# 2646207530/hamer-yolo

Measured on AMD Instinct MI355X. Metric: hands/sec (HaMeR ViT-H/16 + decoder + MANO forward; detector bypassed), higher is better.
Workload: dtype fp16; 1 GPU; BASELINE configs[1]: batch=64 synthetic 256x256 crops per GPU, HaMeR ViT-H/16 + 6-layer decoder + MANO, 16-bit MFMA (fp16 operands), crops resident in HBM; batch_per_gpu=64, global_batch=64, batches_in_flight=2, weights=seeded random-init fp32 master weights, rounded to the operand type at load, parallelism=crop-shard x1

## Files before the change

hamer_yolo_amd/csrc/decoder.hip:

```cpp
#include "common.h"
#include "hamer_hip_internal.h"

namespace {

__global__ __launch_bounds__(256) void linear_f32_kernel(const float* __restrict__ x, int ldx,
                                                         const float* __restrict__ W, int ldw,
                                                         const float* __restrict__ bias, const float* resid, int ldr,
                                                         float* out, int ldo, int M, int N, int K, int act) {
  __shared__ f32x4_t part[4][64];
  const int lane = threadIdx.x & 63, wave = threadIdx.x >> 6;
  const int n0 = blockIdx.x * 16, m0 = blockIdx.y * 16;
  const int g = lane >> 4, li = lane & 15;
  int mr = m0 + li; mr = mr < M ? mr : M - 1;
  int nr = n0 + li; nr = nr < N ? nr : N - 1;
  const float* xp = x + (size_t)mr * ldx + 4 * g;
  const float* wp = W + (size_t)nr * ldw + 4 * g;
  f32x4_t acc = f32x4_t{0.f, 0.f, 0.f, 0.f};
  constexpr int PF = 4;
  int kb = wave * 16;
  for (; kb + 64 * (PF - 1) < K; kb += 64 * PF) {
    f32x4_t xv[PF], wv[PF];
#pragma unroll
    for (int p = 0; p < PF; ++p) { xv[p] = *(const f32x4_t*)(xp + kb + 64 * p); wv[p] = *(const f32x4_t*)(wp + kb + 64 * p); }
#pragma unroll
    for (int p = 0; p < PF; ++p)
#pragma unroll
      for (int i = 0; i < 4; ++i) acc = __builtin_amdgcn_mfma_f32_16x16x4f32(wv[p][i], xv[p][i], acc, 0, 0, 0);
  }
  for (; kb < K; kb += 64) {
    const f32x4_t xv = *(const f32x4_t*)(xp + kb);
    const f32x4_t wv = *(const f32x4_t*)(wp + kb);
#pragma unroll
    for (int i = 0; i < 4; ++i) acc = __builtin_amdgcn_mfma_f32_16x16x4f32(wv[i], xv[i], acc, 0, 0, 0);
  }
  part[wave][lane] = acc;
  __syncthreads();
  if (wave != 0) return;
  f32x4_t v = (part[0][lane] + part[1][lane]) + (part[2][lane] + part[3][lane]);
  const int m = m0 + li, n = n0 + 4 * g;
  if (m >= M || n >= N) return;
  if (bias) v += *(const f32x4_t*)(bias + n);
  if (act == 1) {
#pragma unroll
    for (int r = 0; r < 4; ++r) v[r] = gelu_erf(v[r]);
  }
  if (resid) v += *(const f32x4_t*)(resid + (size_t)m * ldr + n);
  *(f32x4_t*)(out + (size_t)m * ldo + n) = v;
}

constexpr int CA_MAXT = 256;

template <class E>
__global__ __launch_bounds__(64) void cross_attention_kernel(const float* __restrict__ q, const E* __restrict__ kv,
                                                             int ldkv, int k_off, int v_off, float* __restrict__ out,
                                                             int B, int tokens, int heads, float scale) {
  __shared__ float ps[CA_MAXT];
  __shared__ float qs[64];
  typedef __attribute__((ext_vector_type(8))) E vec8;
  const int lane = threadIdx.x;
  const int b = blockIdx.x / heads, h = blockIdx.x % heads;
  const int inner = heads * 64;
  qs[lane] = q[(size_t)b * inner + h * 64 + lane];
  __syncthreads();
  const E* kbase = kv + (size_t)b * tokens * ldkv + k_off + h * 64;
// ... 19 lines not shown
        }
      sc[i] = (d0 + d1) * scale;
      mx = fmaxf(mx, sc[i]);
    }
  }
  mx = wave_max(mx);
  float sum = 0.f;
#pragma unroll
  for (int i = 0; i < CA_MAXT / 64; ++i) {
    const int t = lane + 64 * i;
    if (t < tokens) {
      float p;
      if constexpr (sizeof(E) == 4) p = expf(sc[i] - mx);
      else p = __expf(sc[i] - mx);
      ps[t] = p;
      sum += p;
    }
  }
  sum = wave_sum(sum);
  __syncthreads();
  float o[4] = {0.f, 0.f, 0.f, 0.f};
  int t = 0;
  for (; t + 8 <= tokens; t += 8) {
    float v[8];
#pragma unroll
    for (int j = 0; j < 8; ++j) v[j] = (float)vbase[(size_t)(t + j) * ldkv + lane];
#pragma unroll
    for (int j = 0; j < 8; ++j) o[j & 3] = fmaf(ps[t + j], v[j], o[j & 3]);
  }
  for (; t < tokens; ++t) o[0] = fmaf(ps[t], (float)vbase[(size_t)t * ldkv + lane], o[0]);
  out[(size_t)b * inner + h * 64 + lane] = ((o[0] + o[1]) + (o[2] + o[3])) / sum;
}

__global__ void split_head_kernel(const float* __restrict__ head, int ldh, float* __restrict__ pose6d,
                                  float* __restrict__ betas, float* __restrict__ cam, int B) {
  const int i = blockIdx.x * 256 + threadIdx.x;
  if (i >= B * 109) return;
  const int b = i / 109, c = i % 109;
  const float v = head[(size_t)b * ldh + c];
  if (c < 96) pose6d[b * 96 + c] = v;
  else if (c < 106) betas[b * 10 + (c - 96)] = v;
  else cam[b * 3 + (c - 106)] = v;
}

}

extern "C" int hm_linear_f32(const float* x, int ldx, const float* W, int ldw, const float* bias, const float* resid,
                             int ldr, float* out, int ldo, int M, int N, int K, int act, void* stream_) {
  if (!x || !W || !out || M <= 0 || N <= 0 || K <= 0) return hm_set_error(HM_ERR_ARG, "hm_linear_f32: bad arguments");
  if (K % 16 != 0 || N % 4 != 0 || ldx % 4 != 0 || ldw % 4 != 0 || ldo % 4 != 0 || (resid && ldr % 4 != 0))
    return hm_set_error(HM_ERR_ARG, "hm_linear_f32: K % 16, N % 4 and ld % 4 must be 0");
  if (ldx < K || ldw < K || ldo < N) return hm_set_error(HM_ERR_ARG, "hm_linear_f32: leading dimension too small");
  if (((uintptr_t)x | (uintptr_t)W | (uintptr_t)out | (uintptr_t)bias | (uintptr_t)resid) & 15)
    return hm_set_error(HM_ERR_ARG, "hm_linear_f32: pointers must be 16-byte aligned");
  dim3 grid((N + 15) / 16, (M + 15) / 16), block(256);
  HmProfScope prof(HM_K_LINEAR_F32, act, M, N, K, (hipStream_t)stream_);
  hipLaunchKernelGGL(linear_f32_kernel, grid, block, 0, (hipStream_t)stream_, x, ldx, W, ldw, bias, resid, ldr, out, ldo,
                     M, N, K, act);
  return hm_check_launch("hm_linear_f32");
}

extern "C" int hm_cross_attention(const float* q, const void* kv, int ldkv, int k_off, int v_off, float* out, int B,
                                  int tokens, int heads, int dim_head, float scale, int dtype, void* stream_) {
  if (!q || !kv || !out || B <= 0 || heads <= 0) return hm_set_error(HM_ERR_ARG, "hm_cross_attention: bad arguments");
  if (dim_head != 64 || tokens <= 0 || tokens > CA_MAXT)
    return hm_set_error(HM_ERR_ARG, "hm_cross_attention: dim_head must be 64 and tokens <= 256");
  if (ldkv % 8 != 0 || k_off % 8 != 0 || v_off % 8 != 0 || ((uintptr_t)kv & 15))
    return hm_set_error(HM_ERR_ARG, "hm_cross_attention: kv rows must be 16-byte aligned");
  if (dtype == HM_DTYPE_F32 && ((uintptr_t)kv & 31)) return hm_set_error(HM_ERR_ARG, "hm_cross_attention: fp32 kv rows must be 32-byte aligned");
  dim3 grid(B * heads), block(64);
  hipStream_t s = (hipStream_t)stream_;
  HmProfScope prof(HM_K_CROSS_ATTN, 0, B, tokens, heads, s);
  if (dtype == HM_DTYPE_BF16)
    hipLaunchKernelGGL(cross_attention_kernel<__bf16>, grid, block, 0, s, q, (const __bf16*)kv, ldkv, k_off, v_off, out, B, tokens, heads, scale);
  else if (dtype == HM_DTYPE_F16)
    hipLaunchKernelGGL(cross_attention_kernel<_Float16>, grid, block, 0, s, q, (const _Float16*)kv, ldkv, k_off, v_off, out, B, tokens, heads, scale);
  else if (dtype == HM_DTYPE_F32)
    hipLaunchKernelGGL(cross_attention_kernel<float>, grid, block, 0, s, q, (const float*)kv, ldkv, k_off, v_off, out, B, tokens, heads, scale);
  else
    return hm_set_error(HM_ERR_ARG, "hm_cross_attention: bad dtype");
  return hm_check_launch("hm_cross_attention");
}

int hm_split_head(const float* head, int ldh, float* pose6d, float* betas, float* cam, int B, hipStream_t s) {
  hipLaunchKernelGGL(split_head_kernel, dim3((B * 109 + 255) / 256), dim3(256), 0, s, head, ldh, pose6d, betas, cam, B);
  return hm_check_launch("hm_split_head");
}
```

hamer_yolo_amd/csrc/forward.hip:

```cpp
#include "common.h"
#include <stdlib.h>
#include "hamer_hip_internal.h"

int hm_split_head(const float* head, int ldh, float* pose6d, float* betas, float* cam, int B, hipStream_t s);

namespace {

inline size_t align256(size_t x) { return (x + 255) & ~(size_t)255; }

struct Layout {
  size_t patches, x, h, qkv, att, mlp, kv, xd, hd, t1, t2, head, stats, rowstats, hs, mlps, atts, partials, total;
  size_t x2, tsize, tmetric, tindex;
  int ksplit_proj, ksplit_fc2;
};

int pick_split_k(int M, int N, int K) {
  const int tiles = ((M + 127) / 128) * ((N + 127) / 128), nk = K / 64;
  if (M > 2048 || N < 512 || K % 64 != 0 || tiles * 2 > 256) return 1;
  int want = 256 / tiles;
  if (want > 8) want = 8;
  if (want > nk) want = nk;
  while (want > 1 && nk % want != 0) --want;
  return want;
}
// ... 253 lines not shown
      }
      HM_TRY(hm_layernorm_mx8(x, b.ln2_g, b.ln2_b, h, hs, M, D, w->vit_eps, stream));
      HM_TRY(gemm8(h, hs, D, b.fc1_w8, b.fc1_ws, w->mlp_dim, mlp, w->mlp_dim, b.fc1_b, HM_EPI_GELU_MX8, nullptr, mlps));
      HM_TRY(gemm8(mlp, mlps, w->mlp_dim, b.fc2_w8, b.fc2_ws, D, x, D, b.fc2_b, HM_EPI_RESID_F32, x, nullptr));
    } else if (fold) {
      HM_TRY(gemm(h, D, b.qkv_w, D, 3 * D, qkv, 3 * D, b.qkv_bias_ln, HM_EPI_LN_STORE, nullptr, 0, 0, b.qkv_colsum));
      HM_TRY(hm_vit_attention(qkv, att, B, tokens, w->heads, D / w->heads, scale, dt, stream));
      HM_TRY(gemm(att, D, b.proj_w, D, D, x, D, b.proj_b, HM_EPI_RESID_LN, x, D, 0, b.ln2_g));
      HM_TRY(gemm(h, D, b.fc1_w, D, w->mlp_dim, mlp, w->mlp_dim, b.fc1_bias_ln, HM_EPI_LN_GELU, nullptr, 0, 0, b.fc1_colsum));
      if (i + 1 < w->depth) HM_TRY(gemm(mlp, w->mlp_dim, b.fc2_w, w->mlp_dim, D, x, D, b.fc2_b, HM_EPI_RESID_LN, x, D, 0, w->blocks[i + 1].ln1_g));
      else HM_TRY(gemm(mlp, w->mlp_dim, b.fc2_w, w->mlp_dim, D, x, D, b.fc2_b, HM_EPI_RESID_F32, x, D, 0));
    } else {
      if (i == 0) {
        HM_TRY(hm_layernorm(x, b.ln1_g, b.ln1_b, h, dt, M, D, w->vit_eps, stream));
        HM_TRY(probe(h, D, M, 0, D, 0));
      }
      HM_TRY(gemm(h, D, b.qkv_w, D, 3 * D, qkv, 3 * D, b.qkv_b, HM_EPI_STORE, nullptr, 0, 0));
      for (int c = 0; c < 3; ++c) HM_TRY(probe(qkv, 3 * D, M, c * D, D, 6 * i + 1 + c));
      HM_TRY(hm_vit_attention(qkv, att, B, tokens, w->heads, D / w->heads, b.attn_scale_mul != 0.f ? scale * b.attn_scale_mul : scale, dt, stream));
      HM_TRY(resid_gemm_ln(att, D, b.proj_w, b.proj_b, L.ksplit_proj, b.ln2_g, b.ln2_b, h));
      HM_TRY(probe(h, D, M, 0, D, 6 * i + 4));
      HM_TRY(gemm(h, D, b.fc1_w, D, w->mlp_dim, mlp, w->mlp_dim, b.fc1_b, HM_EPI_GELU, nullptr, 0, 0, nullptr, b.gelu_out_scale));
      HM_TRY(probe(mlp, w->mlp_dim, M, 0, w->mlp_dim, 6 * i + 5));
      const bool last = i + 1 == w->depth;
      HM_TRY(resid_gemm_ln(mlp, w->mlp_dim, b.fc2_w, b.fc2_b, L.ksplit_fc2, last ? w->last_g : w->blocks[i + 1].ln1_g,
                           last ? w->last_b : w->blocks[i + 1].ln1_b, last ? tok : h));
      HM_TRY(probe(last ? tok : h, D, M, 0, D, 6 * (i + 1)));
    }
  }
  if (fold || fp8) HM_TRY(hm_layernorm(x, w->last_g, w->last_b, tok, dt, M, D, w->vit_eps, stream));
  }

  const int dim = w->dec_dim, inner = w->dec_heads * w->dec_dim_head, ldkv = w->dec_depth * 2 * inner;
  {
    hm_gemm_args g{};
    g.X = tok; g.W = w->kv_w; g.C = kv; g.M = B * ctx_tokens; g.N = ldkv; g.K = D; g.ldx = D; g.ldw = D; g.ldc = ldkv;
    g.epilogue = dt == HM_DTYPE_F32 ? HM_EPI_F32 : HM_EPI_STORE; g.dtype = dt;
    if (dt == HM_DTYPE_F32) HM_TRY(hm_gemm_f32(&g, stream));
    else HM_TRY(hm_gemm(&g, stream));
    for (int i = 0; i < w->dec_depth; ++i) {
      HM_TRY(probe(kv, ldkv, B * ctx_tokens, i * 2 * inner, inner, 6 * w->depth + 1 + 2 * i));
      HM_TRY(probe(kv, ldkv, B * ctx_tokens, i * 2 * inner + inner, inner, 6 * w->depth + 2 + 2 * i));
    }
  }
  float *xd = (float*)(ws + L.xd), *hd = (float*)(ws + L.hd), *t1 = (float*)(ws + L.t1), *t2 = (float*)(ws + L.t2);
  HM_TRY(hm_broadcast_rows(w->token0, xd, B, dim, stream));
  const float dscale = 1.0f / sqrtf((float)w->dec_dim_head);
  for (int i = 0; i < w->dec_depth; ++i) {
    const hm_dec_layer& l = w->layers[i];
    HM_TRY(hm_layernorm(xd, l.ln0_g, l.ln0_b, hd, HM_OUT_F32, B, dim, w->dec_eps, stream));
    if (l.sa_w) {
      HM_TRY(hm_linear_f32(hd, dim, l.sa_w, dim, l.sa_out_b, xd, dim, xd, dim, B, dim, dim, 0, stream));
    } else {
      HM_TRY(hm_linear_f32(hd, dim, l.sa_v_w, dim, nullptr, nullptr, 0, t1, inner, B, inner, dim, 0, stream));
      HM_TRY(hm_linear_f32(t1, inner, l.sa_out_w, inner, l.sa_out_b, xd, dim, xd, dim, B, dim, inner, 0, stream));
    }
    HM_TRY(hm_layernorm(xd, l.ln1_g, l.ln1_b, hd, HM_OUT_F32, B, dim, w->dec_eps, stream));
    HM_TRY(hm_linear_f32(hd, dim, l.ca_q_w, dim, nullptr, nullptr, 0, t1, inner, B, inner, dim, 0, stream));
    HM_TRY(hm_cross_attention(t1, kv, ldkv, i * 2 * inner, i * 2 * inner + inner, t2, B, ctx_tokens, w->dec_heads,
                              w->dec_dim_head, l.ca_scale_mul != 0.f ? dscale * l.ca_scale_mul : dscale, dt, stream));
    HM_TRY(hm_linear_f32(t2, inner, l.ca_out_w, inner, l.ca_out_b, xd, dim, xd, dim, B, dim, inner, 0, stream));
    HM_TRY(hm_layernorm(xd, l.ln2_g, l.ln2_b, hd, HM_OUT_F32, B, dim, w->dec_eps, stream));
    HM_TRY(hm_linear_f32(hd, dim, l.ff1_w, dim, l.ff1_b, nullptr, 0, t1, w->dec_mlp, B, w->dec_mlp, dim, 1, stream));
    HM_TRY(hm_linear_f32(t1, w->dec_mlp, l.ff2_w, w->dec_mlp, l.ff2_b, xd, dim, xd, dim, B, dim, w->dec_mlp, 0, stream));
  }
  float* head = (float*)(ws + L.head);
  HM_TRY(hm_linear_f32(xd, dim, w->head_w, dim, w->head_b, nullptr, 0, head, 112, B, 112, dim, 0, stream));
  HM_TRY(hm_split_head(head, 112, out->pose6d, out->betas, out->cam, B, (hipStream_t)stream));
  return hm_mano_forward(&w->mano, out->pose6d, out->betas, out->cam, out->rotmats, out->verts, out->joints, out->cam_t,
                         out->kp2d, B, w->focal_length, w->image_size, stream);
}
```

hamer_yolo_amd/csrc/status.hip:

```cpp
#include <stdio.h>
#include <string.h>
#include "common.h"
#include "hamer_hip_internal.h"

static thread_local char g_err[512] = "";

int hm_set_error(int code, const char* msg) {
  snprintf(g_err, sizeof(g_err), "%s", msg ? msg : "");
  return code;
}

int hm_check_launch(const char* what) {
  hipError_t e = hipGetLastError();
  if (e == hipSuccess) return HM_OK;
  snprintf(g_err, sizeof(g_err), "%s: %s", what, hipGetErrorString(e));
  return HM_ERR_HIP;
}

int hm_device_cu_count(void) {
  static std::mutex mu;
  static int cus[64] = {0};
  int dev = 0;
  if (hipGetDevice(&dev) != hipSuccess) return -1;
  std::lock_guard<std::mutex> lock(mu);
  if (dev < 64 && cus[dev] > 0) return cus[dev];
  int n = 0;
  if (hipDeviceGetAttribute(&n, hipDeviceAttributeMultiprocessorCount, dev) != hipSuccess) return -1;
  if (dev < 64) cus[dev] = n;
  return n;
}

#include <atomic>
static std::atomic<int> g_opts[HM_OPT_COUNT];
int hm_option(int key) {
  return (key >= 0 && key < HM_OPT_COUNT) ? g_opts[key].load(std::memory_order_relaxed) : 0;
}
extern "C" int hm_get_option(int key) { return hm_option(key); }
extern "C" int hm_option_count(void) { return HM_OPT_COUNT; }
extern "C" int hm_set_option(int key, int value) {
  if (key < 0 || key >= HM_OPT_COUNT) return hm_set_error(HM_ERR_ARG, "hm_set_option: unknown key");
  if (value < 0) return hm_set_error(HM_ERR_ARG, "hm_set_option: value must be >= 0");
  if ((key == HM_OPT_PX_GRID || key == HM_OPT_FP8P_GRID) && value != 0 && (value < 8 || value % 8 != 0))
    return hm_set_error(HM_ERR_ARG, "hm_set_option: a persistent grid is 0 (default) or a multiple of the 8 XCDs");
  if (key == HM_OPT_GEMM_STAGGER && value > 4)
    return hm_set_error(HM_ERR_ARG, "hm_set_option: HM_OPT_GEMM_STAGGER is 0 (default), 1 (lockstep), 2 (staggered), 3 or 4 (one kernel staggered)");
  g_opts[key].store(value, std::memory_order_relaxed);
  return HM_OK;
}

extern "C" int hm_version(void) { return HM_VERSION; }
extern "C" const char* hm_last_error_string(void) { return g_err; }
```

hamer_yolo_amd/lib.py:

```python
from __future__ import annotations

import ctypes as C
import os

HERE = os.path.dirname(os.path.abspath(__file__))
LIB_PATH = os.path.join(HERE, "libhamer_hip.so")

HM_DTYPE_BF16, HM_DTYPE_F16, HM_OUT_F32 = 0, 1, 2
HM_DTYPE_F32 = 2
HM_EPI_STORE, HM_EPI_GELU, HM_EPI_RESID_F32, HM_EPI_F32, HM_EPI_SILU = 0, 1, 2, 3, 4
HM_EPI_RESID_LN, HM_EPI_LN_STORE, HM_EPI_LN_GELU, HM_EPI_GELU_MX8 = 5, 6, 7, 8
HM_VERSION = 402
OPTION_NAMES = ("HM_OPT_PX_GRID", "HM_OPT_FP8P_GRID", "HM_OPT_FP8_ONE_TILE", "HM_OPT_FP8P_RESID", "HM_OPT_TOME_NO_SPLITK",
                "HM_OPT_TOME_SCALAR_ATTENTION", "HM_OPT_RESID_IN_EPILOGUE", "HM_OPT_CONV_TILE", "HM_OPT_CONV_SPLITK",
                "HM_OPT_PX_LDS_EPILOGUE", "HM_OPT_CONV_DIRECT", "HM_OPT_GEMM_TILE_RULE", "HM_OPT_CONV_KGROUPS",
                "HM_OPT_CONV_GENERAL_LOADER", "HM_OPT_CONV_STEM_PAIR", "HM_OPT_ATT_GRID", "HM_OPT_GEMM_STAGGER")
globals().update({_n: _i for _i, _n in enumerate(OPTION_NAMES)})

EXPORTS = [
    "hm_version", "hm_last_error_string", "hm_gemm", "hm_layernorm", "hm_vit_attention", "hm_patch_im2col",
    "hm_linear_f32", "hm_broadcast_rows", "hm_cross_attention", "hm_mano_forward", "hm_crop_box_from_bbox",
    "hm_crop_batch", "hm_hamer_workspace_bytes", "hm_hamer_forward", "hm_prof_begin", "hm_prof_collect", "hm_prof_end",
    "hm_conv2d_nhwc", "hm_conv2d_stem_pair", "hm_maxpool_nhwc", "hm_upsample2x_nhwc", "hm_letterbox_plan_make", "hm_letterbox_tables",
    "hm_letterbox", "hm_yolo_decode", "hm_nms_workspace_bytes", "hm_yolo_nms", "hm_yolo_run", "hm_gemm_set_variant", "hm_gemm_set_group_m", "hm_ln_finalize", "hm_layernorm_accum", "hm_gemm_fp8", "hm_layernorm_mx8", "hm_vit_attention_mx8", "hm_nchw3_to_nhwc8", "hm_gap_linear",
    "hm_tome_index_bytes", "hm_tome_attention", "hm_tome_merge", "hm_set_option", "hm_get_option", "hm_tome_merge_metric", "hm_conv_splitk_bytes", "hm_yolo_decode_batch", "hm_letterbox_batch",
    "hm_option_count", "hm_gemm_px_grid", "hm_absmax16", "hm_mesh_overlay_workspace_bytes", "hm_mesh_overlay",
    "hm_sar_saigb", "hm_sar_graph_mix", "hm_sar_linear", "hm_sar_softargmax", "hm_sar_postprocess",
    "hm_conv2d_f32_relu", "hm_nchw3_to_nhwc8_f32", "hm_gap_linear_f32", "hm_sar_saigb_f32", "hm_sar_graph_mix_f32", "hm_sar_linear_f32",
    "hm_gemm_f32", "hm_vit_attention_f32",
    "hm_dwconv7_ln", "hm_ln_patchify2", "hm_stem4_im2col", "hm_sar_saigb_ch",
    "hm_mesh_render_workspace_bytes", "hm_mesh_render",
    "hm_attention_grid",
    "hm_crop_aa_box_from_bbox", "hm_crop_batch_aa",
    "hm_pose_eval",
    "hm_skeleton_overlay_workspace_bytes", "hm_skeleton_overlay",
    "hm_det_match", "hm_det_ap_workspace_bytes", "hm_det_ap", "hm_det_ap_curve",
    "hm_nms_batch_workspace_bytes", "hm_yolo_nms_batch",
    "hm_tta_sizes", "hm_tta_tables", "hm_tta_scale", "hm_yolo_decode_batch_tta",
    "hm_mesh_score", "hm_pck_auc_workspace_bytes", "hm_pck_auc",
    "hm_mask_score_workspace_bytes", "hm_mask_score",
]
KIND_NAMES = ["gemm", "layernorm", "attention", "im2col", "linear_f32", "cross_attn", "mano", "crop", "conv", "other"]


class HipLibraryError(RuntimeError):
    pass


vp, fp = C.c_void_p, C.c_void_p


class GemmArgs(C.Structure):
    _fields_ = [("X", vp), ("W", vp), ("C", vp), ("bias", vp), ("resid", vp),
                ("M", C.c_int), ("N", C.c_int), ("K", C.c_int),
                ("ldx", C.c_int), ("ldw", C.c_int), ("ldc", C.c_int), ("ldr", C.c_int),
                ("resid_mod", C.c_int), ("epilogue", C.c_int), ("dtype", C.c_int),
                ("ln_gamma", vp), ("ln_xg", vp), ("ln_stats", vp), ("ln_colsum", vp), ("k_split", C.c_int), ("out_scale", C.c_float)]


class GemmFp8Args(C.Structure):
    _fields_ = [("X8", vp), ("x_scales", vp), ("W8", vp), ("w_scale", vp), ("C", vp), ("bias", vp), ("resid", vp),
                ("out_scales", vp), ("M", C.c_int), ("N", C.c_int), ("K", C.c_int), ("ldx", C.c_int), ("ldw", C.c_int),
                ("ldc", C.c_int), ("ldr", C.c_int), ("epilogue", C.c_int), ("out_dtype", C.c_int)]


class ManoModel(C.Structure):
    _fields_ = [("v_template", vp), ("shapedirs", vp), ("posedirs", vp), ("J_regressor", vp), ("lbs_weights", vp),
                ("n_verts", C.c_int)]


class CropBox(C.Structure):
    _fields_ = [("m0", C.c_double), ("m4", C.c_double), ("x0", C.c_int32), ("y0", C.c_int32),
                ("flip", C.c_int32), ("reserved", C.c_int32)]
# ... 97 lines not shown
class HamerOutputs(C.Structure):
    _fields_ = [(n, vp) for n in ("pose6d", "betas", "cam", "rotmats", "verts", "joints", "cam_t", "kp2d", "tokens")]


_lib = None


def load() -> C.CDLL:
    global _lib
    if _lib is not None:
        return _lib
    if not os.path.exists(LIB_PATH):
        raise HipLibraryError(
            f"{LIB_PATH} not found: build it with `python -m hamer_yolo_amd.build` (hipcc, gfx950). "
            "There is no CPU fallback for the hot path.")
    try:
        import torch
    except ImportError:
        pass
    try:
        lib = C.CDLL(LIB_PATH)
    except OSError as e:
        raise HipLibraryError(f"cannot load {LIB_PATH}: {e}") from e
    i, f, d = C.c_int, C.c_float, C.c_double
    lib.hm_version.restype = i
    lib.hm_last_error_string.restype = C.c_char_p
    lib.hm_gemm.argtypes = [C.POINTER(GemmArgs), vp]
    lib.hm_layernorm.argtypes = [vp, vp, vp, vp, i, i, i, f, vp]
    lib.hm_vit_attention.argtypes = [vp, vp, i, i, i, i, f, i, vp]
    lib.hm_patch_im2col.argtypes = [vp, vp, i, i, i, i, i, i, i, i, vp]
    lib.hm_linear_f32.argtypes = [vp, i, vp, i, vp, vp, i, vp, i, i, i, i, i, vp]
    lib.hm_broadcast_rows.argtypes = [vp, vp, i, i, vp]
    lib.hm_cross_attention.argtypes = [vp, vp, i, i, i, vp, i, i, i, i, f, i, vp]
    lib.hm_mano_forward.argtypes = [C.POINTER(ManoModel), vp, vp, vp, vp, vp, vp, vp, vp, i, f, f, vp]
    lib.hm_crop_box_from_bbox.argtypes = [d, d, d, i, i, C.POINTER(CropBox)]
    lib.hm_crop_batch.argtypes = [vp, i, i, vp, vp, i, i, C.POINTER(C.c_float), C.POINTER(C.c_float), vp]
    lib.hm_crop_aa_box_from_bbox.argtypes = [d, d, d, i, i, C.POINTER(CropAaBox), C.POINTER(C.c_float)]
    lib.hm_crop_batch_aa.argtypes = [vp, i, i, vp, vp, vp, i, i, C.POINTER(C.c_float), C.POINTER(C.c_float), vp]
    lib.hm_hamer_workspace_bytes.argtypes = [C.POINTER(HamerWeights), i]
    lib.hm_hamer_workspace_bytes.restype = C.c_size_t
    lib.hm_hamer_forward.argtypes = [C.POINTER(HamerWeights), vp, i, C.POINTER(HamerOutputs), vp, C.c_size_t, vp]
    lib.hm_ln_finalize.argtypes = [vp, vp, i, i, C.c_float, vp]
    lib.hm_gemm_fp8.argtypes = [C.POINTER(GemmFp8Args), vp]
    lib.hm_layernorm_mx8.argtypes = [vp, vp, vp, vp, vp, i, i, C.c_float, vp]
    lib.hm_vit_attention_mx8.argtypes = [vp, vp, vp, i, i, i, i, C.c_float, vp]
    lib.hm_nchw3_to_nhwc8.argtypes = [vp, vp, i, i, i, i, vp]
    lib.hm_gap_linear.argtypes = [vp, i, i, vp, C.c_float, vp, vp, i, i, vp]
    lib.hm_layernorm_accum.argtypes = [vp, vp, i, vp, vp, vp, vp, i, i, i, C.c_float, vp]
    lib.hm_absmax16.argtypes = [vp, i, i, i, i, i, vp, vp]
    lib.hm_conv2d_nhwc.argtypes = [C.POINTER(ConvArgs), vp]
    lib.hm_conv_splitk_bytes.argtypes = [C.POINTER(ConvArgs)]
    lib.hm_conv2d_stem_pair.argtypes = [C.POINTER(ConvArgs), C.POINTER(ConvArgs), vp]
    lib.hm_conv_splitk_bytes.restype = C.c_size_t
    lib.hm_maxpool_nhwc.argtypes = [vp, i, vp, i, i, i, i, i, i, i, i, i, vp]
    lib.hm_upsample2x_nhwc.argtypes = [vp, i, vp, i, i, i, i, i, i, vp]
    lib.hm_letterbox_plan_make.argtypes = [i, i, i, i, C.POINTER(LetterboxPlan)]
    lib.hm_letterbox_tables.argtypes = [C.POINTER(LetterboxPlan), C.POINTER(C.c_int32)]
    lib.hm_letterbox.argtypes = [vp, C.POINTER(LetterboxPlan), vp, vp, i, vp, vp]
    lib.hm_letterbox_batch.argtypes = [vp, C.c_size_t, i, C.POINTER(LetterboxPlan), vp, vp, i, vp]
    lib.hm_yolo_decode.argtypes = [vp, i, vp, i, i, i, i, f, C.POINTER(C.c_float), vp]
    lib.hm_yolo_decode_batch.argtypes = [vp, i, vp, i, i, i, i, f, C.POINTER(C.c_float), i, C.c_size_t, vp]
    lib.hm_tta_sizes.argtypes = [i, i, d, i, C.POINTER(C.c_int)]
    lib.hm_tta_tables.argtypes = [i, i, d, i, i, C.POINTER(C.c_int32)]
    lib.hm_tta_scale.argtypes = [vp, vp, vp, i, i, i, d, i, i, vp]
    lib.hm_yolo_decode_batch_tta.argtypes = [vp, i, vp, i, i, i, i, f, C.POINTER(C.c_float), i, C.c_size_t, f, i, f, vp]
    lib.hm_nms_workspace_bytes.argtypes = [i]
# ... 137 lines not shown
```

include/hamer_hip.h:

```cpp
#ifndef HAMER_HIP_H
#define HAMER_HIP_H
#include <stddef.h>
#include <stdint.h>

#ifdef __cplusplus
extern "C" {
#endif

#define HM_VERSION 402

enum { HM_DTYPE_BF16 = 0, HM_DTYPE_F16 = 1,
       HM_DTYPE_F32 = 2  };

enum {
  HM_EPI_STORE = 0,
  HM_EPI_GELU = 1,
  HM_EPI_RESID_F32 = 2,
  HM_EPI_F32 = 3,
  HM_EPI_SILU = 4,
  HM_EPI_RESID_LN = 5,
  HM_EPI_LN_STORE = 6,
  HM_EPI_LN_GELU = 7,
  HM_EPI_GELU_MX8 = 8,
  HM_EPI_RELU = 9,
// ... 11 lines not shown
  int resid_mod;
  int epilogue;
  int dtype;
  const float* ln_gamma;
  void* ln_xg;
  float* ln_stats;
  const float* ln_colsum;
  int k_split;
  float out_scale;
} hm_gemm_args;

int hm_gemm(const hm_gemm_args* args, void* stream);
int hm_ln_finalize(const float* partials, float* row_stats, int M, int D, float eps, void* stream);
int hm_gemm_set_variant(int variant);
int hm_gemm_set_group_m(int group_m);
enum {
  HM_OPT_PX_GRID = 0,
  HM_OPT_FP8P_GRID = 1,
  HM_OPT_FP8_ONE_TILE = 2,
  HM_OPT_FP8P_RESID = 3,
  HM_OPT_TOME_NO_SPLITK = 4,
  HM_OPT_TOME_SCALAR_ATTENTION = 5,
  HM_OPT_RESID_IN_EPILOGUE = 6,
  HM_OPT_CONV_TILE = 7,
  HM_OPT_CONV_SPLITK = 8,
  HM_OPT_PX_LDS_EPILOGUE = 9,
  HM_OPT_CONV_DIRECT = 10,
  HM_OPT_GEMM_TILE_RULE = 11,
  HM_OPT_CONV_KGROUPS = 12,
  HM_OPT_CONV_GENERAL_LOADER = 13,
  HM_OPT_CONV_STEM_PAIR = 14,
  HM_OPT_ATT_GRID = 15,
  HM_OPT_GEMM_STAGGER = 16,
  HM_OPT_COUNT = 17
};
int hm_set_option(int key, int value);
int hm_get_option(int key);
int hm_option_count(void);
int hm_gemm_px_grid(int tiles, int cus);
int hm_attention_grid(int items, int cus);

typedef struct hm_gemm_fp8_args {
  const void* X8; const void* x_scales;
  const void* W8; const float* w_scale;
  void* C; const float* bias; const float* resid; void* out_scales;
  int M, N, K, ldx, ldw, ldc, ldr;
  int epilogue;
  int out_dtype;
} hm_gemm_fp8_args;
int hm_gemm_fp8(const hm_gemm_fp8_args* args, void* stream);
int hm_layernorm_mx8(const float* x, const float* gamma, const float* beta, void* out8, void* out_scales, int M, int D,
                     float eps, void* stream);

#define HM_OUT_F32 2
int hm_layernorm(const float* x, const float* gamma, const float* beta, void* out, int out_dtype,
                 int M, int D, float eps, void* stream);
int hm_layernorm_accum(float* x, const float* partials, int n_partials, const float* bias, const float* gamma,
                       const float* beta, void* out, int out_dtype, int M, int D, float eps, void* stream);
int hm_absmax16(const void* x, int ld, int M, int col0, int ncols, int dtype, float* slot, void* stream);

int hm_vit_attention(const void* qkv, void* out, int B, int tokens, int heads, int head_dim, float scale,
                     int dtype, void* stream);

size_t hm_tome_index_bytes(int B);
int hm_tome_attention(const void* qkv, const float* size, void* out, int B, int tokens, int heads, int head_dim, float scale,
                      int dtype, void* stream);
int hm_tome_merge(const void* qkv, const float* x, const float* size, float* x_out, float* size_out, float* metric_ws,
                  int* index_ws, int B, int tokens, int r, int heads, int head_dim, int D, int dtype, void* stream);
int hm_tome_merge_metric(const float* metric, int ld_metric, int lo_off, const float* x, const float* size, float* x_out,
                         float* size_out, int* index_ws, int B, int tokens, int r, int D, void* stream);

int hm_vit_attention_mx8(const void* qkv, void* out8, void* out_scales, int B, int tokens, int heads, int head_dim, float scale,
                         void* stream);

int hm_patch_im2col(const float* img, void* patches, int B, int img_h, int img_w_full, int x0, int win_w,
                    int patch, int pad, int dtype, void* stream);

int hm_linear_f32(const float* x, int ldx, const float* W, int ldw, const float* bias, const float* resid, int ldr,
                  float* out, int ldo, int M, int N, int K, int act, void* stream);


int hm_broadcast_rows(const float* vec, float* out, int B, int D, void* stream);

int hm_cross_attention(const float* q, const void* kv, int ldkv, int k_off, int v_off, float* out, int B, int tokens,
                       int heads, int dim_head, float scale, int dtype, void* stream);

typedef struct hm_mano_model {
  const float* v_template;
  const float* shapedirs;
  const float* posedirs;
  const float* J_regressor;
  const float* lbs_weights;
  int n_verts;
} hm_mano_model;

int hm_mano_forward(const hm_mano_model* model, const float* pose6d, const float* betas, const float* cam,
                    float* rotmats, float* verts, float* joints, float* cam_t, float* kp2d, int B,
                    float focal_length, float image_size, void* stream);

typedef struct hm_crop_box {
  double m0, m4;
  int32_t x0, y0;
  int32_t flip;
  int32_t reserved;
} hm_crop_box;

int hm_crop_box_from_bbox(double cx, double cy, double size, int flip, int P, hm_crop_box* out);

int hm_crop_batch(const uint8_t* frame, int H, int W, const hm_crop_box* boxes, float* out, int B, int P,
                  const float* mean3_host, const float* std3_host, void* stream);

#define HM_CROP_AA_MAX_SIGMA 12.0
#define HM_CROP_AA_MAX_RADIUS 48
#define HM_CROP_AA_TAPS (HM_CROP_AA_MAX_RADIUS + 1)
typedef struct hm_crop_aa_box {
  double m0, m4;
  int32_t x0, y0;
  int32_t flip;
// ... 299 lines not shown
```

Before: 3862 hands/s.

## Skip decoder to_kv GEMM by folding K/V projections into cross-attention

Adds a token-space cross-attention kernel that projects each query through W_k onto the ViT tokens, computes softmax weights directly over the raw tokens, and applies W_v after the weighted token sum. This removes the large per-layer to_kv GEMM over all B*tokens rows when the decoder has a single query token. It also adds an optional linear kernel with a fused LayerNorm prologue, selected by option value 2. The token tail is on by default for 16-bit, non-ToMe, non-fp8 configurations. In exchange, each cross-attention block rereads every token row twice and the W_k/W_v slices for its head pair, with a different floating-point summation order.

```diff
diff --git a/hamer_yolo_amd/csrc/decoder.hip b/hamer_yolo_amd/csrc/decoder.hip
--- a/hamer_yolo_amd/csrc/decoder.hip
+++ b/hamer_yolo_amd/csrc/decoder.hip
@@ -3,10 +3,24 @@
 
 namespace {
 
+constexpr int LIN_LN_MAXJ = 8;
+__device__ __forceinline__ float ln_squares(f32x4_t d, bool one_piece) {
+  if (one_piece) return __fadd_rn(fmaf(d[0], d[0], __fmul_rn(d[1], d[1])), fmaf(d[2], d[2], __fmul_rn(d[3], d[3])));
+  return __fadd_rn(__fadd_rn(__fmul_rn(d[0], d[0]), __fmul_rn(d[1], d[1])), __fadd_rn(__fmul_rn(d[2], d[2]), __fmul_rn(d[3], d[3])));
+}
+__device__ __forceinline__ f32x4_t ln_apply(f32x4_t x, float mean, float rstd, f32x4_t g, f32x4_t b) {
+  const f32x4_t d = x - mean;
+  f32x4_t y;
+#pragma unroll
+  for (int e = 0; e < 4; ++e) y[e] = fmaf(__fmul_rn(d[e], rstd), g[e], b[e]);
+  return y;
+}
+template <bool LN>
 __global__ __launch_bounds__(256) void linear_f32_kernel(const float* __restrict__ x, int ldx,
                                                          const float* __restrict__ W, int ldw,
                                                          const float* __restrict__ bias, const float* resid, int ldr,
-                                                         float* out, int ldo, int M, int N, int K, int act) {
+                                                         float* out, int ldo, int M, int N, int K, int act,
+                                                         const float* __restrict__ ln_g, const float* __restrict__ ln_b, float eps) {
   __shared__ f32x4_t part[4][64];
   const int lane = threadIdx.x & 63, wave = threadIdx.x >> 6;
   const int n0 = blockIdx.x * 16, m0 = blockIdx.y * 16;
@@ -15,6 +29,40 @@
   int nr = n0 + li; nr = nr < N ? nr : N - 1;
   const float* xp = x + (size_t)mr * ldx + 4 * g;
   const float* wp = W + (size_t)nr * ldw + 4 * g;
+  float mean = 0.f, rstd = 1.f;
+  const float *gp = nullptr, *bp = nullptr;
+  if constexpr (LN) {
+    __shared__ float lnst[16][2];
+    for (int r = 0; r < 4; ++r) {
+      int row = m0 + wave * 4 + r; row = row < M ? row : M - 1;
+      const float* xr = x + (size_t)row * ldx;
+      f32x4_t v[LIN_LN_MAXJ];
+#pragma unroll
+      for (int j = 0; j < LIN_LN_MAXJ; ++j) {
+        const int i = lane * 4 + j * 256;
+        v[j] = f32x4_t{0.f, 0.f, 0.f, 0.f};
+        if (i < K) v[j] = *(const f32x4_t*)(xr + i);
+      }
+      float s = 0.f;
+#pragma unroll
+      for (int j = 0; j < LIN_LN_MAXJ; ++j) s += (v[j][0] + v[j][1]) + (v[j][2] + v[j][3]);
+      const float mu = wave_sum(s) / (float)K;
+      float q = 0.f;
+#pragma unroll
+      for (int j = 0; j < LIN_LN_MAXJ; ++j) {
+        const int i = lane * 4 + j * 256;
+        if (i < K) {
+          const f32x4_t d = v[j] - mu;
+          q += ln_squares(d, K <= 256);
+        }
+      }
+      const float rs = 1.0f / sqrtf(wave_sum(q) / (float)K + eps);
+      if (lane == 0) { lnst[wave * 4 + r][0] = mu; lnst[wave * 4 + r][1] = rs; }
+    }
+    __syncthreads();
+    mean = lnst[li][0]; rstd = lnst[li][1];
+    gp = ln_g + 4 * g; bp = ln_b + 4 * g;
+  }
   f32x4_t acc = f32x4_t{0.f, 0.f, 0.f, 0.f};
   constexpr int PF = 4;
   int kb = wave * 16;
@@ -22,14 +70,20 @@
     f32x4_t xv[PF], wv[PF];
 #pragma unroll
     for (int p = 0; p < PF; ++p) { xv[p] = *(const f32x4_t*)(xp + kb + 64 * p); wv[p] = *(const f32x4_t*)(wp + kb + 64 * p); }
+    if constexpr (LN) {
+#pragma unroll
+      for (int p = 0; p < PF; ++p)
+        xv[p] = ln_apply(xv[p], mean, rstd, *(const f32x4_t*)(gp + kb + 64 * p), *(const f32x4_t*)(bp + kb + 64 * p));
+    }
 #pragma unroll
     for (int p = 0; p < PF; ++p)
 #pragma unroll
       for (int i = 0; i < 4; ++i) acc = __builtin_amdgcn_mfma_f32_16x16x4f32(wv[p][i], xv[p][i], acc, 0, 0, 0);
   }
   for (; kb < K; kb += 64) {
-    const f32x4_t xv = *(const f32x4_t*)(xp + kb);
+    f32x4_t xv = *(const f32x4_t*)(xp + kb);
     const f32x4_t wv = *(const f32x4_t*)(wp + kb);
+    if constexpr (LN) xv = ln_apply(xv, mean, rstd, *(const f32x4_t*)(gp + kb), *(const f32x4_t*)(bp + kb));
 #pragma unroll
     for (int i = 0; i < 4; ++i) acc = __builtin_amdgcn_mfma_f32_16x16x4f32(wv[i], xv[i], acc, 0, 0, 0);
   }
@@ -115,6 +169,251 @@
   out[(size_t)b * inner + h * 64 + lane] = ((o[0] + o[1]) + (o[2] + o[3])) / sum;
 }
 
+constexpr int CT_HPG = 2;
+constexpr int CT_MAXG = 3;
+constexpr int CT_MAXD = CT_MAXG * 64 * 8;
+constexpr int CT_WAVES = 8, CT_THREADS = CT_WAVES * 64;
+constexpr int CT_TU = 4;
+static_assert(CT_WAVES == 8 && 64 % (4 * CT_WAVES) == 0, "slab hand-over and the W_v row walk are written for 8 waves");
+
+template <int CTRL>
+__device__ __forceinline__ float dpp_lane(float v) {
+  return __builtin_bit_cast(float, __builtin_amdgcn_mov_dpp(__builtin_bit_cast(int, v), CTRL, 0xF, 0xF, true));
+}
+__device__ __forceinline__ float wave_sum_tree(float v) {
+  v += dpp_lane<0xB1>(v);
+  v += dpp_lane<0x4E>(v);
+  v += dpp_lane<0x141>(v);
+  v += dpp_lane<0x140>(v);
+  v += __shfl_xor(v, 16, 64);
+  v += __shfl_xor(v, 32, 64);
+  return v;
+}
+
+template <class E>
+__global__ __launch_bounds__(CT_THREADS) void cross_attention_tokens_kernel(const float* __restrict__ q, const E* __restrict__ tok,
+                                                                            const E* __restrict__ wk, const E* __restrict__ wv,
+                                                                            float* __restrict__ out, int B, int tokens, int heads,
+                                                                            int D, float scale) {
+  typedef __attribute__((ext_vector_type(8))) E vec8;
+  __shared__ float buf[4 * CT_HPG * CT_MAXD];
+  __shared__ float sc[CT_HPG][CA_MAXT];
+  __shared__ float ps[CA_MAXT][CT_HPG];
+  __shared__ float qs[CT_HPG * 64];
+  __shared__ float os[CT_HPG * 64];
+  __shared__ float ssum[CT_HPG];
+  const int tid = threadIdx.x, lane = tid & 63, wave = tid >> 6;
+  const int b = blockIdx.x % B, h0 = (blockIdx.x / B) * CT_HPG;
+  const int inner = heads * 64, G = D >> 3;
+  if (tid < CT_HPG * 64) qs[tid] = q[(size_t)b * inner + h0 * 64 + tid];
+  __syncthreads();
+
+  for (int item = tid; item < CT_HPG * G; item += CT_THREADS) {
+    const int hh = item / G, g = item - hh * G;
+    const E* wr = wk + (size_t)(h0 + hh) * 64 * D + g * 8;
+    float a[8] = {0.f, 0.f, 0.f, 0.f, 0.f, 0.f, 0.f, 0.f};
+    for (int j = 0; j < 64; j += 16) {
+      vec8 w8[16];
+#pragma unroll
+      for (int u = 0; u < 16; ++u) w8[u] = *(const vec8*)(wr + (size_t)(j + u) * D);
+#pragma unroll
+      for (int u = 0; u < 16; ++u) {
+        const float qj = qs[hh * 64 + j + u];
+#pragma unroll
+        for (int e = 0; e < 8; ++e) a[e] = fmaf(qj, (float)w8[u][e], a[e]);
+      }
+    }
+    float* dst = buf + hh * D + g * 8;
+    *(f32x4_t*)dst = f32x4_t{a[0], a[1], a[2], a[3]};
+    *(f32x4_t*)(dst + 4) = f32x4_t{a[4], a[5], a[6], a[7]};
+  }
+  __syncthreads();
+
+  auto load_row = [&](const E* row, vec8 (&x)[CT_MAXG]) {
+#pragma unroll
+    for (int i = 0; i < CT_MAXG; ++i) {
+      const int g = lane + 64 * i;
+#pragma unroll
+      for (int e = 0; e < 8; ++e) x[i][e] = (E)0.f;
+      if (g < G) x[i] = *(const vec8*)(row + g * 8);
+    }
+  };
+  auto load_lds = [&](const float* src, float (&r)[CT_MAXG][8]) {
+#pragma unroll
+    for (int i = 0; i < CT_MAXG; ++i) {
+      const int g = lane + 64 * i;
+#pragma unroll
+      for (int e = 0; e < 8; ++e) r[i][e] = 0.f;
+      if (g < G) {
+        const f32x4_t lo = *(const f32x4_t*)(src + g * 8), hi = *(const f32x4_t*)(src + g * 8 + 4);
+#pragma unroll
+        for (int e = 0; e < 4; ++e) { r[i][e] = lo[e]; r[i][4 + e] = hi[e]; }
+      }
+    }
+  };
+  auto dot_row = [&](const vec8 (&x)[CT_MAXG], const float (&r)[CT_MAXG][8]) {
+    float d0 = 0.f, d1 = 0.f;
+#pragma unroll
+    for (int i = 0; i < CT_MAXG; ++i)
+#pragma unroll
+      for (int e = 0; e < 8; e += 2) {
+        d0 = fmaf(r[i][e], (float)x[i][e], d0);
+        d1 = fmaf(r[i][e + 1], (float)x[i][e + 1], d1);
+      }
+    return d0 + d1;
+  };
+  const E* tb = tok + (size_t)b * tokens * D;
+  constexpr int STEP = CT_WAVES * CT_TU;
+  auto load_step = [&](int t, vec8 (&x)[CT_TU][CT_MAXG]) {
+#pragma unroll
+    for (int u = 0; u < CT_TU; ++u) {
+      const int tu = t + CT_WAVES * u;
+      load_row(tb + (size_t)(tu < tokens ? tu : t) * D, x[u]);
+    }
+  };
+
+  {
+    float qr[CT_HPG][CT_MAXG][8];
+#pragma unroll
+    for (int hh = 0; hh < CT_HPG; ++hh) load_lds(buf + hh * D, qr[hh]);
+    vec8 cur[CT_TU][CT_MAXG], nxt[CT_TU][CT_MAXG];
+    if (wave < tokens) load_step(wave, cur);
+    for (int t = wave; t < tokens; t += STEP) {
+      if (t + STEP < tokens) load_step(t + STEP, nxt);
+#pragma unroll
+      for (int u = 0; u < CT_TU; ++u) {
+        const int tu = t + CT_WAVES * u;
+#pragma unroll
+        for (int hh = 0; hh < CT_HPG; ++hh) {
+          const float s = wave_sum_tree(dot_row(cur[u], qr[hh])) * scale;
+          if (lane == 0 && tu < tokens) sc[hh][tu] = s;
+        }
+      }
+#pragma unroll
+      for (int u = 0; u < CT_TU; ++u)
+#pragma unroll
+        for (int i = 0; i < CT_MAXG; ++i) cur[u][i] = nxt[u][i];
+    }
+  }
+  __syncthreads();
+
+  if (wave < CT_HPG) {
+    float s[CA_MAXT / 64];
+    float mx = -3.0e38f;
+#pragma unroll
+    for (int i = 0; i < CA_MAXT / 64; ++i) {
+      const int t = lane + 64 * i;
+      s[i] = t < tokens ? sc[wave][t] : -3.0e38f;
+      mx = fmaxf(mx, s[i]);
+    }
+    mx = wave_max(mx);
+    float sum = 0.f;
+#pragma unroll
+    for (int i = 0; i < CA_MAXT / 64; ++i) {
+      const int t = lane + 64 * i;
+      if (t < tokens) {
+        const float p = __expf(s[i] - mx);
+        ps[t][wave] = p;
+        sum += p;
+      }
+    }
+    sum = wave_sum(sum);
+    if (lane == 0) ssum[wave] = sum;
+  }
+  __syncthreads();
+
+  {
+    float acc[CT_HPG][CT_MAXG][8];
+#pragma unroll
+    for (int hh = 0; hh < CT_HPG; ++hh)
+#pragma unroll
+      for (int i = 0; i < CT_MAXG; ++i)
+#pragma unroll
+        for (int e = 0; e < 8; ++e) acc[hh][i][e] = 0.f;
+    vec8 cur[CT_TU][CT_MAXG], nxt[CT_TU][CT_MAXG];
+    if (wave < tokens) load_step(wave, cur);
+    for (int t = wave; t < tokens; t += STEP) {
+      if (t + STEP < tokens) load_step(t + STEP, nxt);
+#pragma unroll
+      for (int u = 0; u < CT_TU; ++u) {
+        const int tu = t + CT_WAVES * u;
+        if (tu < tokens) {
+#pragma unroll
+          for (int hh = 0; hh < CT_HPG; ++hh) {
+            const float p = ps[tu][hh];
+#pragma unroll
+            for (int i = 0; i < CT_MAXG; ++i)
+#pragma unroll
+              for (int e = 0; e < 8; ++e) acc[hh][i][e] = fmaf(p, (float)cur[u][i][e], acc[hh][i][e]);
+          }
+        }
+      }
+#pragma unroll
+      for (int u = 0; u < CT_TU; ++u)
+#pragma unroll
+        for (int i = 0; i < CT_MAXG; ++i) cur[u][i] = nxt[u][i];
+    }
+    float* slab = buf + (size_t)(wave & 3) * CT_HPG * D;
+    if (wave >= 4) {
+#pragma unroll
+      for (int hh = 0; hh < CT_HPG; ++hh)
+#pragma unroll
+        for (int i = 0; i < CT_MAXG; ++i) {
+          const int g = lane + 64 * i;
+          if (g < G) {
+            float* dst = slab + hh * D + g * 8;
+            *(f32x4_t*)dst = f32x4_t{acc[hh][i][0], acc[hh][i][1], acc[hh][i][2], acc[hh][i][3]};
+            *(f32x4_t*)(dst + 4) = f32x4_t{acc[hh][i][4], acc[hh][i][5], acc[hh][i][6], acc[hh][i][7]};
+          }
+        }
+    }
+    __syncthreads();
+    if (wave < 4) {
+#pragma unroll
+      for (int hh = 0; hh < CT_HPG; ++hh)
+#pragma unroll
+        for (int i = 0; i < CT_MAXG; ++i) {
+          const int g = lane + 64 * i;
+          if (g < G) {
+            float* dst = slab + hh * D + g * 8;
+            const f32x4_t lo = *(const f32x4_t*)dst, hi = *(const f32x4_t*)(dst + 4);
+            *(f32x4_t*)dst = f32x4_t{acc[hh][i][0], acc[hh][i][1], acc[hh][i][2], acc[hh][i][3]} + lo;
+            *(f32x4_t*)(dst + 4) = f32x4_t{acc[hh][i][4], acc[hh][i][5], acc[hh][i][6], acc[hh][i][7]} + hi;
+          }
+        }
+    }
+  }
+  __syncthreads();
+  {
+    const int slab = CT_HPG * D;
+    for (int i = tid * 4; i < slab; i += CT_THREADS * 4) {
+      const f32x4_t p0 = *(const f32x4_t*)(buf + i), p1 = *(const f32x4_t*)(buf + slab + i);
+      const f32x4_t p2 = *(const f32x4_t*)(buf + 2 * slab + i), p3 = *(const f32x4_t*)(buf + 3 * slab + i);
+      *(f32x4_t*)(buf + i) = (p0 + p1) + (p2 + p3);
+    }
+  }
+  __syncthreads();
+
+#pragma unroll
+  for (int hh = 0; hh < CT_HPG; ++hh) {
+    float cr[CT_MAXG][8];
+    load_lds(buf + hh * D, cr);
+    const E* wrow = wv + (size_t)(h0 + hh) * 64 * D;
+    for (int j = wave; j < 64; j += 4 * CT_WAVES) {
+      vec8 y[4][CT_MAXG];
+#pragma unroll
+      for (int u = 0; u < 4; ++u) load_row(wrow + (size_t)(j + CT_WAVES * u) * D, y[u]);
+#pragma unroll
+      for (int u = 0; u < 4; ++u) {
+        const float r = wave_sum_tree(dot_row(y[u], cr));
+        if (lane == 0) os[hh * 64 + j + CT_WAVES * u] = r;
+      }
+    }
+  }
+  __syncthreads();
+  if (tid < CT_HPG * 64) out[(size_t)b * inner + h0 * 64 + tid] = os[tid] / ssum[tid >> 6];
+}
+
 __global__ void split_head_kernel(const float* __restrict__ head, int ldh, float* __restrict__ pose6d,
                                   float* __restrict__ betas, float* __restrict__ cam, int B) {
   const int i = blockIdx.x * 256 + threadIdx.x;
@@ -138,9 +437,49 @@
     return hm_set_error(HM_ERR_ARG, "hm_linear_f32: pointers must be 16-byte aligned");
   dim3 grid((N + 15) / 16, (M + 15) / 16), block(256);
   HmProfScope prof(HM_K_LINEAR_F32, act, M, N, K, (hipStream_t)stream_);
-  hipLaunchKernelGGL(linear_f32_kernel, grid, block, 0, (hipStream_t)stream_, x, ldx, W, ldw, bias, resid, ldr, out, ldo,
-                     M, N, K, act);
+  hipLaunchKernelGGL(linear_f32_kernel<false>, grid, block, 0, (hipStream_t)stream_, x, ldx, W, ldw, bias, resid, ldr, out, ldo,
+                     M, N, K, act, (const float*)nullptr, (const float*)nullptr, 0.f);
   return hm_check_launch("hm_linear_f32");
+}
+
+extern "C" int hm_linear_ln_f32(const float* x, int ldx, const float* ln_g, const float* ln_b, float eps, const float* W, int ldw,
+                                const float* bias, const float* resid, int ldr, float* out, int ldo, int M, int N, int K, int act,
+                                void* stream_) {
+  if (!x || !ln_g || !ln_b || !W || !out || M <= 0 || N <= 0 || K <= 0) return hm_set_error(HM_ERR_ARG, "hm_linear_ln_f32: bad arguments");
+  if (K % 16 != 0 || K > 256 * LIN_LN_MAXJ || N % 4 != 0 || ldx % 4 != 0 || ldw % 4 != 0 || ldo % 4 != 0 || (resid && ldr % 4 != 0))
+    return hm_set_error(HM_ERR_ARG, "hm_linear_ln_f32: K % 16, N % 4 and ld % 4 must be 0, K <= 2048");
+  if (ldx < K || ldw < K || ldo < N) return hm_set_error(HM_ERR_ARG, "hm_linear_ln_f32: leading dimension too small");
+  if (((uintptr_t)x | (uintptr_t)W | (uintptr_t)out | (uintptr_t)bias | (uintptr_t)resid | (uintptr_t)ln_g | (uintptr_t)ln_b) & 15)
+    return hm_set_error(HM_ERR_ARG, "hm_linear_ln_f32: pointers must be 16-byte aligned");
+  if (x < out + (size_t)(M - 1) * ldo + N && out < x + (size_t)(M - 1) * ldx + K)
+    return hm_set_error(HM_ERR_ARG, "hm_linear_ln_f32: out overlaps x");
+  dim3 grid((N + 15) / 16, (M + 15) / 16), block(256);
+  HmProfScope prof(HM_K_LINEAR_F32, 2 + act, M, N, K, (hipStream_t)stream_);
+  hipLaunchKernelGGL(linear_f32_kernel<true>, grid, block, 0, (hipStream_t)stream_, x, ldx, W, ldw, bias, resid, ldr, out, ldo,
+                     M, N, K, act, ln_g, ln_b, eps);
+  return hm_check_launch("hm_linear_ln_f32");
+}
+
+extern "C" int hm_cross_attention_tokens(const float* q, const void* tok, const void* wk, const void* wv, float* out, int B,
+                                         int tokens, int heads, int dim_head, int D, float scale, int dtype, void* stream_) {
+  if (!q || !tok || !wk || !wv || !out || B <= 0 || heads <= 0) return hm_set_error(HM_ERR_ARG, "hm_cross_attention_tokens: bad arguments");
+  if (dim_head != 64 || heads % CT_HPG != 0 || tokens <= 0 || tokens > CA_MAXT)
+    return hm_set_error(HM_ERR_ARG, "hm_cross_attention_tokens: dim_head must be 64, heads even and tokens <= 256");
+  if (D <= 0 || D % 8 != 0 || D > CT_MAXD) return hm_set_error(HM_ERR_ARG, "hm_cross_attention_tokens: need D % 8 == 0 and D <= 1536");
+  if (((uintptr_t)tok | (uintptr_t)wk | (uintptr_t)wv) & 15)
+    return hm_set_error(HM_ERR_ARG, "hm_cross_attention_tokens: token and weight rows must be 16-byte aligned");
+  dim3 grid(B * (heads / CT_HPG)), block(CT_THREADS);
+  hipStream_t s = (hipStream_t)stream_;
+  HmProfScope prof(HM_K_CROSS_ATTN, 1, B, tokens, heads, s);
+  if (dtype == HM_DTYPE_BF16)
+    hipLaunchKernelGGL(cross_attention_tokens_kernel<__bf16>, grid, block, 0, s, q, (const __bf16*)tok, (const __bf16*)wk,
+                       (const __bf16*)wv, out, B, tokens, heads, D, scale);
+  else if (dtype == HM_DTYPE_F16)
+    hipLaunchKernelGGL(cross_attention_tokens_kernel<_Float16>, grid, block, 0, s, q, (const _Float16*)tok, (const _Float16*)wk,
+                       (const _Float16*)wv, out, B, tokens, heads, D, scale);
+  else
+    return hm_set_error(HM_ERR_ARG, "hm_cross_attention_tokens: bad dtype (the 16-bit routes only)");
+  return hm_check_launch("hm_cross_attention_tokens");
 }
 
 extern "C" int hm_cross_attention(const float* q, const void* kv, int ldkv, int k_off, int v_off, float* out, int B,
diff --git a/hamer_yolo_amd/csrc/forward.hip b/hamer_yolo_amd/csrc/forward.hip
--- a/hamer_yolo_amd/csrc/forward.hip
+++ b/hamer_yolo_amd/csrc/forward.hip
@@ -309,7 +309,10 @@
   }
 
   const int dim = w->dec_dim, inner = w->dec_heads * w->dec_dim_head, ldkv = w->dec_depth * 2 * inner;
-  {
+  const int tail_opt = hm_option(HM_OPT_DECODER_TAIL);
+  const bool tok_tail = dt != HM_DTYPE_F32 && !w->tome_r && !fp8 && !rs && tail_opt != 1 && w->dec_dim_head == 64 &&
+                        w->dec_heads % 2 == 0 && ctx_tokens <= 256 && D % 8 == 0 && D <= 1536 && dim % 16 == 0 && dim <= 2048;
+  if (!tok_tail) {
     hm_gemm_args g{};
     g.X = tok; g.W = w->kv_w; g.C = kv; g.M = B * ctx_tokens; g.N = ldkv; g.K = D; g.ldx = D; g.ldw = D; g.ldc = ldkv;
     g.epilogue = dt == HM_DTYPE_F32 ? HM_EPI_F32 : HM_EPI_STORE; g.dtype = dt;
@@ -323,6 +326,35 @@
   float *xd = (float*)(ws + L.xd), *hd = (float*)(ws + L.hd), *t1 = (float*)(ws + L.t1), *t2 = (float*)(ws + L.t2);
   HM_TRY(hm_broadcast_rows(w->token0, xd, B, dim, stream));
   const float dscale = 1.0f / sqrtf((float)w->dec_dim_head);
+  if (tok_tail) {
+    auto ln_linear = [&](const float* xin, const float* g, const float* bt, const float* W, const float* bias, const float* resid,
+                         float* o, int ldo, int N, int act) {
+      if (tail_opt == 2)
+        return hm_linear_ln_f32(xin, dim, g, bt, w->dec_eps, W, dim, bias, resid, dim, o, ldo, B, N, dim, act, stream);
+      HM_TRY(hm_layernorm(xin, g, bt, hd, HM_OUT_F32, B, dim, w->dec_eps, stream));
+      return hm_linear_f32(hd, dim, W, dim, bias, resid, dim, o, ldo, B, N, dim, act, stream);
+    };
+    const size_t esz = 2;
+    for (int i = 0; i < w->dec_depth; ++i) {
+      const hm_dec_layer& l = w->layers[i];
+      float* xs = xd == (float*)(ws + L.xd) ? (float*)(ws + L.hd) : (float*)(ws + L.xd);
+      if (tail_opt != 2) xs = xd;
+      if (l.sa_w) {
+        HM_TRY(ln_linear(xd, l.ln0_g, l.ln0_b, l.sa_w, l.sa_out_b, xd, xs, dim, dim, 0));
+        xd = xs;
+      } else {
+        HM_TRY(ln_linear(xd, l.ln0_g, l.ln0_b, l.sa_v_w, nullptr, nullptr, t1, inner, inner, 0));
+        HM_TRY(hm_linear_f32(t1, inner, l.sa_out_w, inner, l.sa_out_b, xd, dim, xd, dim, B, dim, inner, 0, stream));
+      }
+      HM_TRY(ln_linear(xd, l.ln1_g, l.ln1_b, l.ca_q_w, nullptr, nullptr, t1, inner, inner, 0));
+      const char* kw = (const char*)w->kv_w + (size_t)i * 2 * inner * D * esz;
+      HM_TRY(hm_cross_attention_tokens(t1, tok, kw, kw + (size_t)inner * D * esz, t2, B, ctx_tokens, w->dec_heads, w->dec_dim_head, D,
+                                       l.ca_scale_mul != 0.f ? dscale * l.ca_scale_mul : dscale, dt, stream));
+      HM_TRY(hm_linear_f32(t2, inner, l.ca_out_w, inner, l.ca_out_b, xd, dim, xd, dim, B, dim, inner, 0, stream));
+      HM_TRY(ln_linear(xd, l.ln2_g, l.ln2_b, l.ff1_w, l.ff1_b, nullptr, t1, w->dec_mlp, w->dec_mlp, 1));
+      HM_TRY(hm_linear_f32(t1, w->dec_mlp, l.ff2_w, w->dec_mlp, l.ff2_b, xd, dim, xd, dim, B, dim, w->dec_mlp, 0, stream));
+    }
+  } else {
   for (int i = 0; i < w->dec_depth; ++i) {
     const hm_dec_layer& l = w->layers[i];
     HM_TRY(hm_layernorm(xd, l.ln0_g, l.ln0_b, hd, HM_OUT_F32, B, dim, w->dec_eps, stream));
@@ -341,6 +373,7 @@
     HM_TRY(hm_linear_f32(hd, dim, l.ff1_w, dim, l.ff1_b, nullptr, 0, t1, w->dec_mlp, B, w->dec_mlp, dim, 1, stream));
     HM_TRY(hm_linear_f32(t1, w->dec_mlp, l.ff2_w, w->dec_mlp, l.ff2_b, xd, dim, xd, dim, B, dim, w->dec_mlp, 0, stream));
   }
+  }
   float* head = (float*)(ws + L.head);
   HM_TRY(hm_linear_f32(xd, dim, w->head_w, dim, w->head_b, nullptr, 0, head, 112, B, 112, dim, 0, stream));
   HM_TRY(hm_split_head(head, 112, out->pose6d, out->betas, out->cam, B, (hipStream_t)stream));
diff --git a/hamer_yolo_amd/csrc/status.hip b/hamer_yolo_amd/csrc/status.hip
--- a/hamer_yolo_amd/csrc/status.hip
+++ b/hamer_yolo_amd/csrc/status.hip
@@ -44,6 +44,8 @@
     return hm_set_error(HM_ERR_ARG, "hm_set_option: a persistent grid is 0 (default) or a multiple of the 8 XCDs");
   if (key == HM_OPT_GEMM_STAGGER && value > 4)
     return hm_set_error(HM_ERR_ARG, "hm_set_option: HM_OPT_GEMM_STAGGER is 0 (default), 1 (lockstep), 2 (staggered), 3 or 4 (one kernel staggered)");
+  if (key == HM_OPT_DECODER_TAIL && value > 2)
+    return hm_set_error(HM_ERR_ARG, "hm_set_option: HM_OPT_DECODER_TAIL is 0 (default), 1 (to_kv GEMM tail) or 2 (token tail, LayerNorms inside the linears)");
   g_opts[key].store(value, std::memory_order_relaxed);
   return HM_OK;
 }
diff --git a/hamer_yolo_amd/lib.py b/hamer_yolo_amd/lib.py
--- a/hamer_yolo_amd/lib.py
+++ b/hamer_yolo_amd/lib.py
@@ -14,7 +14,8 @@
 OPTION_NAMES = ("HM_OPT_PX_GRID", "HM_OPT_FP8P_GRID", "HM_OPT_FP8_ONE_TILE", "HM_OPT_FP8P_RESID", "HM_OPT_TOME_NO_SPLITK",
                 "HM_OPT_TOME_SCALAR_ATTENTION", "HM_OPT_RESID_IN_EPILOGUE", "HM_OPT_CONV_TILE", "HM_OPT_CONV_SPLITK",
                 "HM_OPT_PX_LDS_EPILOGUE", "HM_OPT_CONV_DIRECT", "HM_OPT_GEMM_TILE_RULE", "HM_OPT_CONV_KGROUPS",
-                "HM_OPT_CONV_GENERAL_LOADER", "HM_OPT_CONV_STEM_PAIR", "HM_OPT_ATT_GRID", "HM_OPT_GEMM_STAGGER")
+                "HM_OPT_CONV_GENERAL_LOADER", "HM_OPT_CONV_STEM_PAIR", "HM_OPT_ATT_GRID", "HM_OPT_GEMM_STAGGER",
+                "HM_OPT_DECODER_TAIL")
 globals().update({_n: _i for _i, _n in enumerate(OPTION_NAMES)})
 
 EXPORTS = [
@@ -39,6 +40,7 @@
     "hm_tta_sizes", "hm_tta_tables", "hm_tta_scale", "hm_yolo_decode_batch_tta",
     "hm_mesh_score", "hm_pck_auc_workspace_bytes", "hm_pck_auc",
     "hm_mask_score_workspace_bytes", "hm_mask_score",
+    "hm_linear_ln_f32", "hm_cross_attention_tokens",
 ]
 KIND_NAMES = ["gemm", "layernorm", "attention", "im2col", "linear_f32", "cross_attn", "mano", "crop", "conv", "other"]
 
@@ -202,6 +204,8 @@
     lib.hm_linear_f32.argtypes = [vp, i, vp, i, vp, vp, i, vp, i, i, i, i, i, vp]
     lib.hm_broadcast_rows.argtypes = [vp, vp, i, i, vp]
     lib.hm_cross_attention.argtypes = [vp, vp, i, i, i, vp, i, i, i, i, f, i, vp]
+    lib.hm_linear_ln_f32.argtypes = [vp, i, vp, vp, f, vp, i, vp, vp, i, vp, i, i, i, i, i, vp]
+    lib.hm_cross_attention_tokens.argtypes = [vp, vp, vp, vp, vp, i, i, i, i, i, f, i, vp]
     lib.hm_mano_forward.argtypes = [C.POINTER(ManoModel), vp, vp, vp, vp, vp, vp, vp, vp, i, f, f, vp]
     lib.hm_crop_box_from_bbox.argtypes = [d, d, d, i, i, C.POINTER(CropBox)]
     lib.hm_crop_batch.argtypes = [vp, i, i, vp, vp, i, i, C.POINTER(C.c_float), C.POINTER(C.c_float), vp]
diff --git a/include/hamer_hip.h b/include/hamer_hip.h
--- a/include/hamer_hip.h
+++ b/include/hamer_hip.h
@@ -67,7 +67,8 @@
   HM_OPT_CONV_STEM_PAIR = 14,
   HM_OPT_ATT_GRID = 15,
   HM_OPT_GEMM_STAGGER = 16,
-  HM_OPT_COUNT = 17
+  HM_OPT_DECODER_TAIL = 17,
+  HM_OPT_COUNT = 18
 };
 int hm_set_option(int key, int value);
 int hm_get_option(int key);
@@ -113,12 +114,17 @@
 
 int hm_linear_f32(const float* x, int ldx, const float* W, int ldw, const float* bias, const float* resid, int ldr,
                   float* out, int ldo, int M, int N, int K, int act, void* stream);
+int hm_linear_ln_f32(const float* x, int ldx, const float* ln_g, const float* ln_b, float eps, const float* W, int ldw,
+                     const float* bias, const float* resid, int ldr, float* out, int ldo, int M, int N, int K, int act,
+                     void* stream);
 
 
 int hm_broadcast_rows(const float* vec, float* out, int B, int D, void* stream);
 
 int hm_cross_attention(const float* q, const void* kv, int ldkv, int k_off, int v_off, float* out, int B, int tokens,
                        int heads, int dim_head, float scale, int dtype, void* stream);
+int hm_cross_attention_tokens(const float* q, const void* tok, const void* wk, const void* wv, float* out, int B, int tokens,
+                              int heads, int dim_head, int D, float scale, int dtype, void* stream);
 
 typedef struct hm_mano_model {
   const float* v_template;
```

After: 3881 hands/s (median of 5 runs). Within noise of the previous version (+0.5%).
